# quickwit-oss/quickwit

Hardware: NVIDIA H100
Metric: docs_scored_per_sec (higher is better)
Workload: dtype f32+u32

## Files before the change

quickwit_b200/csrc/capi_engine.cpp:

```cpp
#include "engine.h"

#define QW_API_BEGIN try {
#define QW_API_END                                   \
  }                                                  \
  catch (const qw::Error& e) {                       \
    qw::set_last_error(e.what());                    \
    return e.code;                                   \
  }                                                  \
  catch (const std::exception& e) {                  \
    qw::set_last_error(e.what());                    \
    return QWGPU_EINTERNAL;                          \
  }

static qw::Engine& engine_of(qwgpu_ctx* ctx) {
  if (!ctx) qw::fail(QWGPU_EINVALID_ARG, "null context");
  if (!ctx->engine) qw::fail(QWGPU_ENODEVICE, "host-only context: no CUDA device bound (there is no CPU search path)");
  return *ctx->engine;
}

extern "C" {

int qwgpu_init(int device, qwgpu_ctx** out) {
  QW_API_BEGIN
  if (!out) qw::fail(QWGPU_EINVALID_ARG, "null out pointer");
// ... 56 lines not shown
int qwgpu_split_is_resident(qwgpu_ctx* ctx, const char* split_id) {
  if (!ctx || !ctx->engine || !split_id) return 0;
  std::lock_guard<std::mutex> g(ctx->engine->mu);
  return ctx->engine->splits.count(split_id) ? 1 : 0;
}

uint64_t qwgpu_resident_bytes(qwgpu_ctx* ctx) {
  if (!ctx || !ctx->engine) return 0;
  std::lock_guard<std::mutex> g(ctx->engine->mu);
  return ctx->engine->resident;
}

int qwgpu_split_search(qwgpu_ctx* ctx, uint32_t num_splits, const char* const* split_ids,
                       const uint8_t* const* plans, const size_t* plan_lens,
                       qwgpu_split_result* results, int* status) {
  QW_API_BEGIN
  qw::Engine& e = engine_of(ctx);
  std::vector<std::shared_ptr<qw::SplitDev>> sp(num_splits);
  std::vector<const uint8_t*> pl(plans, plans + num_splits);
  std::vector<size_t> ln(plan_lens, plan_lens + num_splits);
  for (uint32_t i = 0; i < num_splits; i++) sp[i] = e.find(split_ids[i]);
  std::vector<qw::SplitOutput> outs;
  qw::BatchStats st;
  e.search(sp, pl, ln, outs, st);
  std::string first_err;
  for (uint32_t i = 0; i < num_splits; i++) {
    qwgpu_split_result& r = results[i];
    memset(&r, 0, sizeof r);
    status[i] = outs[i].status;
    if (outs[i].status) { if (first_err.empty()) first_err = outs[i].error; continue; }
    r.num_hits = outs[i].num_hits;
    r.num_partial_hits = (uint32_t)outs[i].hits.size();
    r.num_agg_cells = (uint32_t)outs[i].cells.size();
    if (!outs[i].hits.empty()) {
      r.hits = (QwHit*)malloc(outs[i].hits.size() * sizeof(QwHit));
      memcpy(r.hits, outs[i].hits.data(), outs[i].hits.size() * sizeof(QwHit));
    }
    if (!outs[i].cells.empty()) {
      r.agg_cells = (QwAggCell*)malloc(outs[i].cells.size() * sizeof(QwAggCell));
      memcpy(r.agg_cells, outs[i].cells.data(), outs[i].cells.size() * sizeof(QwAggCell));
    }
    r.gpu_time_us = st.gpu_time_us;
    r.main_kernel_us = st.main_kernel_us;
    r.num_kernel_launches = st.launches;
    r.exact_fallbacks = st.exact_fallbacks;
    r.postings_scored = outs[i].postings_scored;
    r.algorithmic_bytes = outs[i].algorithmic_bytes;
    r.kernel_mask = st.kernel_mask;
    r.window_docs = st.window_docs;
    r.sample_stride = st.sample_stride;
    r.radix_passes = st.radix_passes;
    r.refined = st.refined;
  }
  if (!first_err.empty()) qw::set_last_error(first_err);
  return 0;
  QW_API_END
}

void qwgpu_split_result_free(qwgpu_split_result* r) {
  if (!r) return;
  free(r->hits);
  free(r->agg_cells);
  r->hits = nullptr;
  r->agg_cells = nullptr;
}

}
```

quickwit_b200/csrc/common.h:

```cpp
#pragma once
#include <cmath>
#include <cstdarg>
#include <cstdint>
#include <cstdio>
#include <cstdlib>
#include <cstring>
#include <stdexcept>
#include <string>
#include <vector>

#include "../../include/qwgpu.h"

namespace qw {

struct Error : std::runtime_error {
  int code;
  Error(int c, const std::string& m) : std::runtime_error(m), code(c) {}
};
[[noreturn]] inline void fail(int code, const char* fmt, ...) {
  char buf[1024];
  va_list ap;
  va_start(ap, fmt);
  vsnprintf(buf, sizeof buf, fmt, ap);
  va_end(ap);
  throw Error(code, buf);
}
void set_last_error(const std::string& msg);

inline uint64_t i64_to_u64(int64_t v) { return (uint64_t)v ^ (1ull << 63); }
inline int64_t u64_to_i64(uint64_t v) { return (int64_t)(v ^ (1ull << 63)); }
inline uint64_t f64_to_u64(double d) {
  uint64_t bits;
  memcpy(&bits, &d, 8);
  return (bits & (1ull << 63)) ? ~bits : (bits ^ (1ull << 63));
}
inline double u64_to_f64(uint64_t v) {
  uint64_t bits = (v & (1ull << 63)) ? (v ^ (1ull << 63)) : ~v;
  double d;
  memcpy(&d, &bits, 8);
  return d;
}

constexpr float BM25_K1 = 1.2f;
constexpr float BM25_B = 0.75f;
inline float bm25_idf(uint64_t doc_freq, uint64_t doc_count) {
  float x = ((float)(doc_count - doc_freq) + 0.5f) / ((float)doc_freq + 0.5f);
  return logf(1.0f + x);
}

struct ImageView {
  const uint8_t* base = nullptr;
  uint64_t len = 0;
  const QwImgHeader* hdr = nullptr;
  const QwImgField* fields = nullptr;
  const QwImgTerm* terms = nullptr;
  const QwImgColumn* columns = nullptr;
  const uint8_t* term_bytes = nullptr;
  const uint8_t* strings = nullptr;
  const uint8_t* data = nullptr;

  void open(const uint8_t* p, uint64_t n) {
    if (n < sizeof(QwImgHeader)) fail(QWGPU_EINVALID_ARG, "split image too small");
    const QwImgHeader* h = (const QwImgHeader*)p;
    if (h->magic != QW_IMG_MAGIC) fail(QWGPU_EINVALID_ARG, "bad split image magic");
    if (h->version != QW_IMG_VERSION) fail(QWGPU_EINVALID_ARG, "split image version %u (this library reads version %u)", h->version, QW_IMG_VERSION);
    if (h->total_len > n) fail(QWGPU_EINVALID_ARG, "split image truncated");
    const uint64_t tl = h->total_len;
    auto inside = [](uint64_t off, uint64_t count, uint64_t size, uint64_t limit) {
// ... 94 lines not shown
```

quickwit_b200/csrc/device_types.h:

```cpp
#pragma once
#include <stddef.h>
#include <stdint.h>

#include "../../include/qwgpu_format.h"

#ifndef QW_THREADS
#define QW_THREADS 512
#endif
#ifndef QW_MIN_BLOCKS_PER_SM
#define QW_MIN_BLOCKS_PER_SM 2
#endif
#define QW_WARPS (QW_THREADS / 32)
#define QW_MAX_INSTR 96
#define QW_MAX_DCOLS 16
#define QW_MAX_DAGGS 8
#define QW_MAX_LEVELS QW_MAX_PLAN_DEPTH
#define QW_MAX_TERMS 64
#define QW_BLK_TAB 160
#define QW_MAX_WBLK 512
#define QW_HIST_BINS 2048
#define QW_DIGIT_BITS 11
#define QW_KEY_BITS 192
#define QW_CAND_CAP 8192
#define QW_MAX_TOPK 4096
// ... 54 lines not shown

struct alignas(16) DKeySpec {
  uint32_t kind[2], order[2], col[2];
  uint32_t rbits[2];
  uint32_t hasbit[2];
  uint32_t doc_bits, total_bits;
  uint32_t top_mode;
  float score_scale;
  uint64_t raw_max[2];
  uint32_t narrow, sh_has[2], sh_r[2], sh_doc;
};
static_assert(sizeof(DKeySpec) % 16 == 0, "uint4-copied struct");
enum { QW_TOP_FULL = 0, QW_TOP_SCORE = 1, QW_TOP_COLUMN = 2, QW_TOP_DOC = 3 };

struct DThresh {
  uint64_t key[3];
  uint32_t prefix_bits;
  uint32_t above;
  uint32_t done;
  uint32_t matched;
};

struct DSplitPlan {
  uint64_t data_base;
  uint32_t num_docs, num_windows;
  uint32_t n_instr, instr_base;
  uint32_t n_cols, col_base;
  uint32_t n_aggs, agg_base;
  uint32_t n_terms, n_levels;
  uint32_t max_hits, scoring;
  uint32_t n_fn_slots, n_cells;
  uint32_t fused_score_root;
  uint32_t fast_aggs;
  uint32_t n_stat_cells, pad1;
  uint64_t fn_off[2];
  uint64_t bm25_tab[2];
  DKeySpec key;
  QwSearchAfter sa;
  uint64_t out_num_hits;
  uint64_t out_hist;
  uint64_t out_cand_count;
  uint64_t out_cands;
  uint64_t out_cells;
  uint64_t out_hits;
  uint64_t out_nhits;
};

static_assert(offsetof(DSplitPlan, key) % 16 == 0 && sizeof(DSplitPlan) % 16 == 0, "DKeySpec is read as uint4");

struct SmemLevel {
  uint32_t req, shd, nt, cnt, msum, ssum;
  uint32_t rsc, pad;
};
struct SmemLayout {
  uint32_t instr, cols, aggs, key, hitq;
  uint32_t rangeq;
  SmemLevel lvl[QW_MAX_LEVELS];
  uint32_t tmp, fn[2];
  uint32_t rng, blkrec, termblk, stage, hist, misc;
  uint32_t l0hist;
  uint32_t total;
};

struct KParams {
  const DSplitPlan* plans;
  const DInstr* instrs;
  const DCol* cols;
// ... 20 lines not shown
```

quickwit_b200/csrc/engine.cu:

```cuda
#include <algorithm>
#include <chrono>
#include <cmath>

#include "engine.h"
#include "kernels.cuh"
#include "union_kernel.cuh"
#include "phrase_kernel.cuh"
#include "driver_kernel.cuh"
#include "agg_kernel.cuh"

namespace qw {

#define CUDA_CHECK(expr)                                                                          \
  do {                                                                                            \
    cudaError_t _e = (expr);                                                                      \
    if (_e != cudaSuccess)                                                                        \
      fail((_e == cudaErrorNoDevice || _e == cudaErrorInsufficientDriver) ? QWGPU_ENODEVICE       \
                                                                           : QWGPU_EINTERNAL,     \
           "CUDA error %s at %s:%d: %s", cudaGetErrorName(_e), __FILE__, __LINE__,               \
           cudaGetErrorString(_e));                                                               \
  } while (0)

uint32_t id_to_fieldnorm(uint8_t id);

// ... 689 lines not shown
  if (rec_l0) L.l0hist = take(QW_HIST_BINS * 4);
  if (rangeq) L.rangeq = take(QW_WARPS * (32 + 32 * 4) * 2);
  L.total = off;
  return L;
}

static qwk::USmem make_union_layout(uint32_t W, bool hist, uint32_t budget) {
  qwk::USmem L;
  memset(&L, 0, sizeof L);
  uint32_t off = 0;
  auto take = [&](uint32_t bytes) { uint32_t o = off; off = (off + bytes + 15) & ~15u; return o; };
  L.score = take(W * 4);
  L.bars = take(8 * (2 * QU_SLOTS + QU_CHAIN));
  if (hist) L.hist = take(QW_HIST_BINS * 4);
  L.cands = take(QU_NCW * QU_CANDS * 8 + QU_NCW * 4);
  const uint32_t fixed = QU_MAXBLK * 16 + QU_MAX_TERMS * 16 + 32 + QU_PAD;
  uint32_t cap = budget > off + QU_SLOTS * (fixed + 2048) ? ((budget - off) / QU_SLOTS - fixed) & ~15u : 2048;
  if (const char* e = getenv("QWGPU_UCAP")) cap = (uint32_t)atoi(e) & ~15u;
  L.cap = cap;
  L.payload = 0;
  L.recs = cap + QU_PAD;
  L.ttab = L.recs + QU_MAXBLK * 16;
  L.hdr = L.ttab + QU_MAX_TERMS * 16;
  L.slot_stride = L.hdr + 48;
  L.slot0 = take(QU_SLOTS * L.slot_stride);
  L.total = off;
  return L;
}

void Engine::search(const std::vector<std::shared_ptr<SplitDev>>& sp, const std::vector<const uint8_t*>& plans,
                    const std::vector<size_t>& plan_lens, std::vector<SplitOutput>& outs, BatchStats& stats,
                    const MergeSpec* merge, std::vector<MergedHit>* merged, const GatherSpec* gather, std::vector<RankHeader>* rank_headers) {
  const uint32_t n_in = (uint32_t)sp.size();
  outs.assign(n_in, SplitOutput());
  static const bool trace = getenv("QWGPU_TRACE") != nullptr;
  using tclock = std::chrono::steady_clock;
  const auto t_begin = tclock::now();
  CUDA_CHECK(cudaSetDevice(device));
  std::vector<Lowered> low;
  std::vector<uint32_t> idx;
  low.reserve(n_in);
  for (uint32_t i = 0; i < n_in; i++) {
    try {
      if (!sp[i]) fail(QWGPU_ENOTFOUND, "split not registered");
      Lowered L;
      lower_plan(L, *sp[i], plans[i], plan_lens[i]);
      low.push_back(std::move(L));
      idx.push_back(i);
    } catch (const Error& e) {
      outs[i].status = e.code;
      outs[i].error = e.what();
    }
  }
  const uint32_t n = (uint32_t)low.size();
  if (n == 0) {
    if (merge && merged && gather && gather->allgather && gather->world > 1 && rank_headers && merge->k) {
      const size_t rec = 64 + (size_t)merge->k * sizeof(qwk::DMergedHit), W8 = (size_t)gather->world;
      uint8_t *d = nullptr;
      const size_t o_recv = 256 * ((rec + 255) / 256), o_fin = o_recv + 256 * ((W8 * rec + 255) / 256), o_cut = o_fin + 256 * ((16 + rec + 255) / 256), o_hd = o_cut + 1024, total = o_hd + W8 * 64;
      CUDA_CHECK(cudaMalloc(&d, total));
      cudaStream_t st0 = nullptr;
      CUDA_CHECK(cudaStreamCreateWithFlags(&st0, cudaStreamNonBlocking));
      CUDA_CHECK(cudaMemsetAsync(d, 0, total, st0));
      qwk::DRankHeader h;
      memset(&h, 0, sizeof h);
      h.attempted = gather->attempted; h.successful = gather->successful; h.n_failed = gather->n_failed;
      CUDA_CHECK(cudaMemcpyAsync(d, &h, sizeof h, cudaMemcpyHostToDevice, st0));
// ... 160 lines not shown
  fw_all[0] = fw_smp[0] = 0;
  for (uint32_t i = 0; i < n; i++) {
    uint32_t nw = low[i].P.num_windows, phase = stride > 1 ? i % stride : 0;
    fw_all[i + 1] = fw_all[i] + nw;
    if (use_union) nw = low[i].empty ? 0 : (low[i].P.num_docs + W_h - 1) / W_h;
    if (edge_sample) {
      uint32_t cnt = 0;
      for (uint32_t w = 0; w < nw; w++) {
        const bool edge = w == 0 || w + 1 == nw, strided = w % stride == phase;
        if (edge || strided) { sample_win.push_back(w | (edge ? 0x80000000u : 0u)); cnt++; }
      }
      fw_smp[i + 1] = fw_smp[i] + cnt;
    } else fw_smp[i + 1] = fw_smp[i] + (nw > phase ? (nw - phase + stride - 1) / stride : 0);
  }
  uint32_t n_phrases = 0, phrase_blocks = 0;
  for (auto& L : low)
    for (size_t k = 0; k < L.phrases.size(); k++) { n_phrases++; phrase_blocks += L.instrs[L.phrase_instr[k]].n; }
  auto al = [](size_t x) { return (x + 255) & ~(size_t)255; };
  size_t o_plans = 0, o_instr = al(o_plans + n * sizeof(DSplitPlan)), o_cols = al(o_instr + tot_instr * sizeof(DInstr)),
         o_aggs = al(o_cols + std::max(tot_cols, 1u) * sizeof(DCol)), o_fwa = al(o_aggs + std::max(tot_aggs, 1u) * sizeof(DAgg)),
         o_fws = al(o_fwa + (n + 1) * 4), o_bounds = al(o_fws + (n + 1) * 4), o_rank = al(o_bounds + (size_t)tot_bounds * 8),
         o_smp = al(o_rank + (size_t)n * 4), o_phr = al(o_smp + sample_win.size() * 4), o_fwd = al(o_phr + (size_t)n_phrases * sizeof(DPhrase)),
         o_fwds = al(o_fwd + (use_driver ? (size_t)(n + 1) * 4 : 0)), blob_bytes = al(o_fwds + (use_driver ? (size_t)(n + 1) * 4 : 0));
  const bool do_merge = merge && merged && merge->k > 0 && any_topk && merge->rank.size() == n_in;
  uint32_t kmax = 1;
  for (auto& L : low) kmax = std::max(kmax, L.P.max_hits);
  size_t s_thr = 0, s_hist = al(s_thr + n * sizeof(DThresh)), s_state = al(s_hist + (size_t)n * QW_HIST_BINS * 4),
         s_ctr = al(s_state + (size_t)n * 4), s_wmax = al(s_ctr + 64 * 4), s_cand = al(s_wmax + (rec_l0 ? (size_t)fw_all[n] * 2 : 0)),
         s_hits = al(s_cand + (any_topk ? (size_t)n * QW_CAND_CAP * 24 : 0)),
         s_cut = al(s_hits + (do_merge ? (size_t)n * kmax * sizeof(QwHit) : 0)),
         s_grecv = al(s_cut + (size_t)std::max<uint32_t>(n, 64) * 4 + 1024),
         s_vblk = al(s_grecv + (gather && gather->world > 1 && do_merge ? (size_t)gather->world * (64 + (size_t)merge->k * sizeof(qwk::DMergedHit)) : 0)),
         scratch_bytes = al(s_vblk + (size_t)phrase_blocks * sizeof(VBlk));
  std::vector<size_t> out_off(n + 1);
  out_off[0] = 0;
  for (uint32_t i = 0; i < n; i++)
    out_off[i + 1] = al(out_off[i] + 32 + (do_merge ? 0 : (size_t)low[i].P.max_hits * sizeof(QwHit)) + (size_t)low[i].P.n_cells * sizeof(QwAggCell));
  const size_t o_merged = out_off[n];
  const size_t rec_bytes = do_merge ? 64 + (size_t)merge->k * sizeof(qwk::DMergedHit) : 0;
  const bool do_gather = do_merge && gather && gather->allgather && gather->world > 1 && rank_headers;
  const size_t o_ghdr = al(o_merged + rec_bytes), o_final = al(o_ghdr + (do_gather ? (size_t)gather->world * 64 : 0));
  size_t out_bytes = do_merge ? (do_gather ? al(o_final + 16 + (size_t)merge->k * sizeof(qwk::DMergedHit)) : al(o_merged + rec_bytes)) : out_off[n];

  static const int max_in_flight = getenv("QWGPU_MAX_IN_FLIGHT") ? std::max(1, atoi(getenv("QWGPU_MAX_IN_FLIGHT"))) : 16;
  CallSlot* slot = nullptr;
  {
    std::unique_lock<std::mutex> g(mu);
    cv_admit.wait(g, [&] { return admitted < max_in_flight; });
    admitted++;
    if (!free_slots.empty()) { slot = free_slots.back(); free_slots.pop_back(); }
  }
  struct Admit {
    Engine* e;
    ~Admit() {
      { std::lock_guard<std::mutex> g(e->mu); e->admitted--; }
      e->cv_admit.notify_one();
    }
  } admit{this};
  if (!slot) {
    slot = new CallSlot();
    CUDA_CHECK(cudaStreamCreateWithFlags(&slot->stream, cudaStreamNonBlocking));
    CUDA_CHECK(cudaEventCreate(&slot->ev0));
    CUDA_CHECK(cudaEventCreate(&slot->ev1));
    CUDA_CHECK(cudaEventCreate(&slot->ev2));
    CUDA_CHECK(cudaEventCreate(&slot->ev3));
    CUDA_CHECK(cudaEventCreateWithFlags(&slot->ev_block, cudaEventBlockingSync | cudaEventDisableTiming));
  }
  struct Release {
    Engine* e; CallSlot* s;
    ~Release() {
      cudaStreamSynchronize(s->stream);
      e->in_flight.fetch_sub(1);
      std::lock_guard<std::mutex> g(e->mu);
      e->free_slots.push_back(s);
    }
  } rel{this, slot};
  in_flight.fetch_add(1);
  static const uint32_t spin_limit = getenv("QWGPU_SPIN_LIMIT") ? (uint32_t)atoi(getenv("QWGPU_SPIN_LIMIT")) : std::max(2u, std::thread::hardware_concurrency() / 4);
  auto wait_stream = [&]() {
    if (in_flight.load(std::memory_order_relaxed) > (int)spin_limit) {
      CUDA_CHECK(cudaEventRecord(slot->ev_block, slot->stream));
      CUDA_CHECK(cudaEventSynchronize(slot->ev_block));
    } else CUDA_CHECK(cudaStreamSynchronize(slot->stream));
  };
  size_t want_blob, want_scratch, want_out;
  {
    std::lock_guard<std::mutex> g(mu);
    hw_blob = std::max(hw_blob, blob_bytes); hw_scratch = std::max(hw_scratch, scratch_bytes); hw_out = std::max(hw_out, out_bytes);
    auto sized = [](size_t hw, size_t need) { return hw <= ((size_t)64 << 20) ? hw : need; };
    want_blob = sized(hw_blob, blob_bytes); want_scratch = sized(hw_scratch, scratch_bytes); want_out = sized(hw_out, out_bytes);
  }
  slot->ensure(want_blob, want_scratch, want_out);
  cudaStream_t st = slot->stream;

  uint32_t phr_done = 0, phr_blocks_done = 0;
  for (uint32_t i = 0; i < n; i++) {
    DSplitPlan& P = low[i].P;
    if (P.fast_aggs && (((size_t)P.n_cells * 4 + 7) & ~(size_t)7) + (size_t)P.n_stat_cells * 24 > stage_bytes_for(W)) P.fast_aggs = 0;
    uint8_t* ob = slot->d_out + out_off[i];
    P.out_num_hits = (uint64_t)ob;
    P.out_nhits = (uint64_t)(ob + 16);
    P.out_cand_count = (uint64_t)(ob + 20);
    P.out_hits = do_merge ? (uint64_t)(slot->d_scratch + s_hits + (size_t)i * kmax * sizeof(QwHit)) : (uint64_t)(ob + 32);
    P.out_cells = (uint64_t)(ob + 32 + (do_merge ? 0 : (size_t)P.max_hits * sizeof(QwHit)));
    P.out_hist = (uint64_t)(slot->d_scratch + s_hist + (size_t)i * QW_HIST_BINS * 4);
    P.out_cands = (uint64_t)(slot->d_scratch + s_cand + (size_t)i * QW_CAND_CAP * 24);
    for (size_t k = 0; k < low[i].phrases.size(); k++) {
      DPhrase& ph = low[i].phrases[k];
      DInstr& pin = low[i].instrs[low[i].phrase_instr[k]];
      ph.first_work = phr_blocks_done;
      ph.out = (uint64_t)(slot->d_scratch + s_vblk + (size_t)phr_blocks_done * sizeof(VBlk));
      pin.a = ph.out;
      phr_blocks_done += pin.n;
      memcpy(slot->h_blob + o_phr + (size_t)phr_done++ * sizeof(DPhrase), &ph, sizeof ph);
    }
    memcpy(slot->h_blob + o_plans + i * sizeof(DSplitPlan), &P, sizeof P);
    memcpy(slot->h_blob + o_instr + P.instr_base * sizeof(DInstr), low[i].instrs.data(), P.n_instr * sizeof(DInstr));
    if (P.n_cols) memcpy(slot->h_blob + o_cols + P.col_base * sizeof(DCol), low[i].cols.data(), P.n_cols * sizeof(DCol));
    if (P.fast_aggs)
      for (DAgg& d : low[i].aggs)
        if (d.kind == QW_AGG_HISTOGRAM) d.bounds = (uint64_t)(slot->d_blob + o_bounds) + (low[i].bounds_base + d.bounds) * 8;
    if (P.n_aggs) memcpy(slot->h_blob + o_aggs + P.agg_base * sizeof(DAgg), low[i].aggs.data(), P.n_aggs * sizeof(DAgg));
    if (!low[i].bounds.empty()) memcpy(slot->h_blob + o_bounds + (size_t)low[i].bounds_base * 8, low[i].bounds.data(), low[i].bounds.size() * 8);
  }
  if (do_merge) for (uint32_t i = 0; i < n; i++) ((uint32_t*)(slot->h_blob + o_rank))[i] = merge->rank[idx[i]];
  if (!sample_win.empty()) memcpy(slot->h_blob + o_smp, sample_win.data(), sample_win.size() * 4);
  if (use_driver) { memcpy(slot->h_blob + o_fwd, fw_drv.data(), (n + 1) * 4); memcpy(slot->h_blob + o_fwds, fw_dsm.data(), (n + 1) * 4); }
  memcpy(slot->h_blob + o_fwa, fw_all.data(), (n + 1) * 4);
  memcpy(slot->h_blob + o_fws, fw_smp.data(), (n + 1) * 4);
  CUDA_CHECK(cudaMemcpyAsync(slot->d_blob, slot->h_blob, blob_bytes, cudaMemcpyHostToDevice, st));
  stats.h2d_bytes += blob_bytes;

  KParams kp;
  memset(&kp, 0, sizeof kp);
  kp.plans = (const DSplitPlan*)(slot->d_blob + o_plans);
  kp.instrs = (const DInstr*)(slot->d_blob + o_instr);
  kp.cols = (const DCol*)(slot->d_blob + o_cols);
// ... 62 lines not shown
      if (dynamic_work && n_ctr < 64) u.work_ctr = (uint32_t*)(slot->d_scratch + s_ctr) + n_ctr++;
#ifdef QU_PROFILE
      static unsigned long long* d_prof = nullptr;
      if (!d_prof) CUDA_CHECK(cudaMalloc(&d_prof, 16 * 8));
      if (mode == qwk::MODE_COLLECT) { CUDA_CHECK(cudaMemsetAsync(d_prof, 0, 16 * 8, st)); u.prof = d_prof; }
#endif
      const uint32_t ugrid = std::min<uint32_t>(q.total_work, (uint32_t)(sm_count * QU_MINB) - (do_gather ? 4u : 0u));
      if (mode == qwk::MODE_HIST) qwk::k_union<qwk::MODE_HIST><<<ugrid, QU_THREADS, u.sm.total, st>>>(u);
      else qwk::k_union<qwk::MODE_COLLECT><<<ugrid, QU_THREADS, u.sm.total, st>>>(u);
#ifdef QU_PROFILE
      if (u.prof && getenv("QWGPU_UPROF")) {
        unsigned long long h[16];
        CUDA_CHECK(cudaMemcpyAsync(h, d_prof, sizeof h, cudaMemcpyDeviceToHost, st));
        wait_stream();
        const double np = (double)ugrid, nc = (double)h[15];
        fprintf(stderr, "[uprof] producer/CTA: total %.0f cyc, empty-wait %.0f, phaseA %.0f, window(A+B) %.0f, windows %.1f, slots %.1f | consumer/warp: total %.0f, full-wait %.0f, chain-wait %.0f (end-of-window %.0f), sweep %.0f, block-loop %.0f, blocks %.1f\n",
                h[0] / np, h[1] / np, h[2] / np, h[3] / np, h[4] / np, h[5] / np, h[8] / nc, h[9] / nc, h[10] / nc, h[11] / nc, h[12] / nc, h[13] / nc, h[14] / nc);
      }
#endif
      stats.launches++;
      stats.kernel_mask |= QWGPU_KERNEL_UNION;
      return;
    }
    uint32_t grid = std::min<uint32_t>(q.total_work, (uint32_t)(sm_count * occ));
    if (mode == qwk::MODE_HIST && all_union && old_union && level == 0 && !use_prefix) qwk::k_window<qwk::MODE_HIST, true><<<grid, QW_THREADS, lay.total, st>>>(q);
    else if (mode == qwk::MODE_HIST) qwk::k_window<qwk::MODE_HIST, false><<<grid, QW_THREADS, lay.total, st>>>(q);
    else if (all_union && old_union) qwk::k_window<qwk::MODE_COLLECT, true><<<grid, QW_THREADS, lay.total, st>>>(q);
    else qwk::k_window<qwk::MODE_COLLECT, false><<<grid, QW_THREADS, lay.total, st>>>(q);
    stats.launches++;
    stats.kernel_mask |= QWGPU_KERNEL_WINDOW;
  };
  const uint32_t sel_smem = 3 * 8 * QW_CAND_CAP;
  auto run_collect = [&](uint32_t flags) {
    if (!(flags & F_CANDS_ONLY)) CUDA_CHECK(cudaMemsetAsync(slot->d_out, 0, out_bytes, st));
    CUDA_CHECK(cudaEventRecord(slot->ev2, st));
    launch_window(qwk::MODE_COLLECT, false, 0, 0, flags);
    CUDA_CHECK(cudaEventRecord(slot->ev3, st));
    if (any_topk) { qwk::k_select<<<n, 1024, sel_smem, st>>>(kp.plans, kp.cols); stats.launches++; }
    if (do_merge) {
      uint32_t* d_cut = (uint32_t*)(slot->d_scratch + s_cut);
      const qwk::SrcSplits src{kp.plans, (const uint32_t*)(slot->d_blob + o_rank), do_gather ? 1u : 0u};
      qwk::k_merge_prep<qwk::SrcSplits><<<1, 1024, 0, st>>>(src, n, merge->k, merge->order1, merge->order2, d_cut);
      const uint64_t threads = (uint64_t)n * kmax * 32;
      qwk::k_merge<qwk::SrcSplits><<<(uint32_t)((threads + 255) / 256), 256, 0, st>>>(src, d_cut, n, kmax, merge->k, merge->order1, merge->order2,
                                                          (qwk::DMergedHit*)(slot->d_out + o_merged + 64), (uint32_t*)(slot->d_out + o_merged));
      stats.launches += 2;
    }
    const size_t back = do_gather ? o_ghdr : out_bytes;
    CUDA_CHECK(cudaMemcpyAsync(slot->h_out, slot->d_out, back, cudaMemcpyDeviceToHost, st));
    stats.d2h_bytes += back;
  };
  std::vector<uint32_t> state(n, 0);
  auto verify = [&]() -> bool {
    bool all = true;
    for (uint32_t i = 0; i < n; i++) {
      state[i] = 0;
      if (low[i].P.max_hits == 0) continue;
      const uint8_t* ob = slot->h_out + out_off[i];
      uint64_t eligible = ((const uint64_t*)ob)[1];
      uint32_t cand = *(const uint32_t*)(ob + 20);
      if (cand > QW_CAND_CAP || cand < std::min<uint64_t>(low[i].P.max_hits, eligible)) { state[i] = 1; all = false; }
    }
    return all;
  };

  const auto t_staged = tclock::now();
  CUDA_CHECK(cudaEventRecord(slot->ev0, st));
// ... 75 lines not shown
    qwk::k_rank_header<<<1, 32, 0, st>>>(kp.plans, n, (qwk::DRankHeader*)(slot->d_out + o_merged), gather->attempted, gather->successful, gather->n_failed);
    uint8_t* g_recv = slot->d_scratch + s_grecv;
    if (gather->allgather(gather->comm, slot->d_out + o_merged, g_recv, rec_bytes, (void*)st)) fail(QWGPU_EINTERNAL, "ncclAllGather failed");
    const qwk::SrcGathered gsrc{g_recv, (uint32_t)rec_bytes, 64u};
    uint32_t* g_cut = d_cut + std::max<uint32_t>(n, 64);
    qwk::k_merge_prep<qwk::SrcGathered><<<1, 1024, 0, st>>>(gsrc, (uint32_t)gather->world, merge->k, merge->order1, merge->order2, g_cut);
    const uint64_t gthreads = (uint64_t)gather->world * merge->k * 32;
    qwk::k_merge<qwk::SrcGathered><<<(uint32_t)((gthreads + 255) / 256), 256, 0, st>>>(gsrc, g_cut, (uint32_t)gather->world, merge->k, merge->k, merge->order1, merge->order2,
                                                                                    (qwk::DMergedHit*)(slot->d_out + o_final + 16), (uint32_t*)(slot->d_out + o_final));
    CUDA_CHECK(cudaMemcpy2DAsync(slot->d_out + o_ghdr, 64, g_recv, rec_bytes, 64, (size_t)gather->world, cudaMemcpyDeviceToDevice, st));
    CUDA_CHECK(cudaMemcpyAsync(slot->h_out + o_ghdr, slot->d_out + o_ghdr, out_bytes - o_ghdr, cudaMemcpyDeviceToHost, st));
    CUDA_CHECK(cudaEventRecord(slot->ev1, st));
    wait_stream();
    stats.launches += 4;
    stats.d2h_bytes += out_bytes - o_ghdr;
  }
  CUDA_CHECK(cudaGetLastError());
  {
    float ms = 0;
    cudaEventElapsedTime(&ms, slot->ev0, slot->ev1);
    stats.gpu_time_us += ms * 1000.f;
    add_main();
    stats.main_kernel_us = main_ms * 1000.f;
  }

  const auto t_searched = tclock::now();
  for (uint32_t i = 0; i < n; i++) {
    SplitOutput& o = outs[idx[i]];
    const DSplitPlan& P = low[i].P;
    const uint8_t* ob = slot->h_out + out_off[i];
    o.num_hits = ((const uint64_t*)ob)[0];
    uint32_t nh = *(const uint32_t*)(ob + 16);
    if (!do_merge) {
      o.hits.assign((const QwHit*)(ob + 32), (const QwHit*)(ob + 32) + nh);
      if (P.key.kind[0] == QW_SORT_DOCID) for (auto& h : o.hits) { h.flags &= ~1u; h.v1 = 0; }
    }
    const QwAggCell* c = (const QwAggCell*)(ob + 32 + (do_merge ? 0 : (size_t)P.max_hits * sizeof(QwHit)));
    o.cells.assign(c, c + P.n_cells);
    for (auto& cell : o.cells) cell.min_mapped = ~cell.min_mapped;
    o.postings_scored = low[i].postings;
    uint64_t bytes = low[i].alg_bytes;
    const SplitDev& s = *sp[idx[i]];
    auto col_bytes = [&](uint32_t c, uint64_t probes) {
      const QwImgColumn& ic = s.view.columns[c];
      uint64_t full = ((uint64_t)ic.num_vals * ic.bits + 7) / 8;
      return std::min<uint64_t>(probes * ((ic.bits + 7) / 8), full);
    };
    uint64_t driver = low[i].min_required_df == ~0ull ? P.num_docs : low[i].min_required_df;
    for (auto& rc : low[i].range_cols) bytes += col_bytes(rc.first, driver);
    const QwPlanHeader* ph = (const QwPlanHeader*)plans[idx[i]];
    for (int k = 0; k < 2; k++)
      if (ph->sort[k].kind == QW_SORT_COLUMN && ph->sort[k].column != 0xFFFFFFFFu && P.max_hits) bytes += col_bytes(ph->sort[k].column, o.num_hits);
    const QwAggNode* an = (const QwAggNode*)(plans[idx[i]] + sizeof(QwPlanHeader) + (size_t)ph->num_nodes * sizeof(QwPlanNode));
    for (uint32_t a = 0; a < ph->num_aggs; a++) if (an[a].column != 0xFFFFFFFFu) bytes += col_bytes(an[a].column, o.num_hits);
    o.algorithmic_bytes = bytes;
  }
  if (do_gather) {
    const uint32_t nm = *(const uint32_t*)(slot->h_out + o_final);
    const qwk::DMergedHit* mh = (const qwk::DMergedHit*)(slot->h_out + o_final + 16);
    merged->resize(nm);
    const bool by_doc = low[0].P.key.kind[0] == QW_SORT_DOCID;
    for (uint32_t j = 0; j < nm; j++) {
      MergedHit& m = (*merged)[j];
      m.hit = mh[j].hit; m.split = mh[j].split; m.pad = 0;
      if (by_doc) { m.hit.flags &= ~1u; m.hit.v1 = 0; }
    }
    rank_headers->resize(gather->world);
    memcpy(rank_headers->data(), slot->h_out + o_ghdr, (size_t)gather->world * 64);
  } else if (do_merge) {
    const uint32_t nm = *(const uint32_t*)(slot->h_out + o_merged);
// ... 19 lines not shown
```

quickwit_b200/csrc/engine.h:

```cpp
#pragma once
#include <condition_variable>
#include <atomic>
#include <map>
#include <memory>
#include <mutex>
#include <thread>
#include <string>
#include <vector>

#include "common.h"

namespace qw {

struct SplitDev {
  std::string id;
  std::vector<uint8_t> dir;
  ImageView view;
  uint8_t* d_data = nullptr;
  float* d_tabs = nullptr;
  uint64_t data_len = 0;
  uint64_t last_use = 0;
  int state = 1;
  std::string load_error;
  ~SplitDev();
};

struct CallSlot;

struct SplitOutput {
  uint64_t num_hits = 0;
  std::vector<QwHit> hits;
  std::vector<QwAggCell> cells;
  int status = 0;
  std::string error;
  uint64_t postings_scored = 0;
  uint64_t algorithmic_bytes = 0;
};
struct MergeSpec {
  uint32_t k = 0;
  uint32_t order1 = QW_ORDER_DESC, order2 = QW_ORDER_DESC;
  std::vector<uint32_t> rank;
};
struct MergedHit {
  QwHit hit;
  uint32_t split;
  uint32_t pad;
};
struct RankHeader {
  uint32_t n_hits, pad;
  uint64_t num_hits, attempted, successful, n_failed, reserved[3];
};
struct GatherSpec {
  int world = 1, rank = 0;
  int (*allgather)(void* comm, const void* send, void* recv, size_t bytes, void* stream) = nullptr;
  void* comm = nullptr;
  uint64_t attempted = 0, successful = 0, n_failed = 0;
};
struct BatchStats {
  float gpu_time_us = 0;
  float main_kernel_us = 0;
  uint32_t launches = 0;
  uint32_t exact_fallbacks = 0;
  uint64_t h2d_bytes = 0, d2h_bytes = 0;
  uint32_t kernel_mask = 0;
// ... 49 lines not shown
```

quickwit_b200/csrc/kernels.cuh:

```cuda
#pragma once
#include <cuda_runtime.h>

#include "device_types.h"

namespace qwk {

extern __shared__ __align__(16) uint8_t qw_smem[];

struct Key {
  uint64_t w0, w1, w2;
};

__device__ __forceinline__ bool key_ge(const Key& a, const Key& b) {
  if (a.w0 != b.w0) return a.w0 > b.w0;
  if (a.w1 != b.w1) return a.w1 > b.w1;
  return a.w2 >= b.w2;
}
__device__ __forceinline__ bool key_lt(const Key& a, const Key& b) { return !key_ge(a, b); }

__device__ __forceinline__ void key_put(Key& k, uint32_t pos, uint64_t v, uint32_t nbits) {
  if (nbits == 0) return;
  const uint32_t sh = 192u - pos - nbits, w = sh >> 6, s = sh & 63u;
  const uint64_t lo = v << s, hi = s ? v >> (64u - s) : 0ull;
  if (w == 0) { k.w2 |= lo; k.w1 |= hi; }
  else if (w == 1) { k.w1 |= lo; k.w0 |= hi; }
  else k.w0 |= lo;
}
__device__ __forceinline__ uint64_t key_get(const Key& k, uint32_t pos, uint32_t nbits) {
  if (nbits == 0) return 0;
  const uint32_t sh = 192u - pos - nbits, w = sh >> 6, s = sh & 63u;
  const uint64_t lo = w == 0 ? k.w2 : (w == 1 ? k.w1 : k.w0);
  const uint64_t hi = w == 0 ? k.w1 : (w == 1 ? k.w0 : 0ull);
  const uint64_t v = s ? ((lo >> s) | (hi << (64u - s))) : lo;
  return nbits >= 64 ? v : (v & ((1ull << nbits) - 1));
}
__device__ __forceinline__ uint32_t key_digit(const Key& k, uint32_t level) {
  uint32_t o = level * QW_DIGIT_BITS, word = o >> 6, sh = o & 63;
  uint64_t hi = word == 0 ? k.w0 : (word == 1 ? k.w1 : k.w2);
  uint64_t lo = word == 0 ? k.w1 : (word == 1 ? k.w2 : 0ull);
  uint64_t v = sh ? ((hi << sh) | (lo >> (64 - sh))) : hi;
  return (uint32_t)(v >> (64 - QW_DIGIT_BITS));
}
__device__ __forceinline__ bool key_prefix_eq(const Key& a, const uint64_t* t, uint32_t bits) {
  if (bits == 0) return true;
  uint64_t x0 = a.w0 ^ t[0], x1 = a.w1 ^ t[1], x2 = a.w2 ^ t[2];
  if (bits <= 64) return (x0 >> (64 - bits)) == 0;
  if (x0) return false;
  if (bits <= 128) return (x1 >> (128 - bits)) == 0;
  if (x1) return false;
  return (x2 >> (192 - bits)) == 0;
}

__device__ __forceinline__ uint32_t f32_ordered(float f) {
  uint32_t b = __float_as_uint(f);
  return (b & 0x80000000u) ? ~b : (b | 0x80000000u);
}
__device__ __forceinline__ uint64_t f64_to_u64_dev(double d) {
  uint64_t b = (uint64_t)__double_as_longlong(d);
  return (b & (1ull << 63)) ? ~b : (b ^ (1ull << 63));
}
__device__ __forceinline__ double mapped_to_f64(uint32_t type, uint64_t m) {
  switch (type) {
    case QW_COL_U64: case QW_COL_BOOL: case QW_COL_STR: return (double)m;
    case QW_COL_I64: case QW_COL_DATETIME: return (double)(long long)(m ^ (1ull << 63));
    default: {
      uint64_t bits = (m & (1ull << 63)) ? (m ^ (1ull << 63)) : ~m;
      return __longlong_as_double((long long)bits);
    }
  }
}

__device__ __forceinline__ uint64_t col_raw(const uint8_t* base, const DCol& c, uint64_t idx) {
  if (c.bits == 0) return 0;
  const uint64_t* w = (const uint64_t*)(base + c.values_off);
  uint64_t bitpos = idx * c.bits, wi = bitpos >> 6;
  uint32_t sh = (uint32_t)(bitpos & 63);
  uint64_t v = __ldg(w + wi) >> sh;
  if (sh + c.bits > 64) v |= __ldg(w + wi + 1) << (64 - sh);
  return c.bits == 64 ? v : (v & ((1ull << c.bits) - 1));
}
__device__ __forceinline__ void col_range(const uint8_t* base, const DCol& c, uint32_t d, uint64_t& a, uint64_t& b) {
  if (c.card == QW_CARD_FULL) { a = d; b = (uint64_t)d + 1; return; }
  const uint8_t* ix = base + c.index_off;
  if (c.card == QW_CARD_OPTIONAL) {
    const uint64_t* present = (const uint64_t*)ix;
    const uint32_t* rank = (const uint32_t*)(ix + 8ull * c.nwords64);
    uint64_t word = __ldg(present + (d >> 6));
    if (!((word >> (d & 63)) & 1)) { a = b = 0; return; }
    a = __ldg(rank + (d >> 6)) + __popcll(word & ((1ull << (d & 63)) - 1));
    b = a + 1;
    return;
  }
// ... 209 lines not shown
    const bool in = (uint32_t)j < nvalid && rel[j] < wlen;
    inmask |= (in ? 1u : 0u) << j;
    f[j] = (has_fn && in) ? fn[rel[j]] : 1u;
  }
#pragma unroll
  for (int j = 0; j < 4; j++) {
    const uint32_t t = tf[j];
    float tfn = 0.0f;
    if ((inmask >> j) & 1) {
      if (t < QW_TFF_ROWS) tfn = __ldg(tab + 256 + t * 256 + f[j]);
      else { float tff = (float)t; tfn = __fdiv_rn(tff, __fadd_rn(tff, __ldg(tab + f[j]))); }
    }
    contrib[j] = __fmul_rn(tg.weight, tfn);
  }
}

struct DocKey {
  Key key;
  bool eligible;
};
__device__ __forceinline__ uint32_t score_lin(const DKeySpec& ks, float score, bool desc) {
  const float x = __fmul_rn(score, ks.score_scale);
  const uint32_t l = x >= 1023.0f ? 1023u : (x > 0.0f ? (uint32_t)x : 0u);
  return desc ? l : 1023u - l;
}
__device__ __forceinline__ DocKey doc_key(const DSplitPlan& P, const DKeySpec& ks, const DCol* cols, const uint8_t* base, uint32_t doc, float score) {
  uint32_t has[2] = {0, 0};
  uint64_t v[2] = {0, 0}, r[2] = {0, 0};
#pragma unroll
  for (int i = 0; i < 2; i++) {
    const bool desc = ks.order[i] == QW_ORDER_DESC;
    if (ks.kind[i] == QW_SORT_SCORE) {
      has[i] = 1;
      v[i] = f64_to_u64_dev((double)score);
      const uint32_t o = f32_ordered(score);
      r[i] = desc ? o : ~o;
      if (i == 0) r[i] |= (uint64_t)score_lin(ks, score, desc) << 32;
    } else if (ks.kind[i] == QW_SORT_COLUMN && ks.col[i] != 0xFFFFFFFFu) {
      const DCol& c = cols[ks.col[i]];
      uint64_t a, b;
      col_range(base, c, doc, a, b);
      if (a != b) {
        has[i] = 1;
        const uint64_t raw = col_raw(base, c, a);
        v[i] = c.min_value + c.gcd * raw;
        r[i] = desc ? raw : ks.raw_max[i] - raw;
      }
    }
  }
  const bool desc1 = ks.order[0] == QW_ORDER_DESC;
  const uint32_t docmask = ks.doc_bits >= 32 ? 0xFFFFFFFFu : ((1u << ks.doc_bits) - 1);
  DocKey out;
  out.key = Key{0, 0, 0};
  const uint32_t docr = desc1 ? doc : docmask - doc;
  if (ks.narrow) {
    out.key.w0 = ((uint64_t)(has[0] & ks.hasbit[0]) << ks.sh_has[0]) | (r[0] << ks.sh_r[0]) |
                 ((uint64_t)(has[1] & ks.hasbit[1]) << ks.sh_has[1]) | (r[1] << ks.sh_r[1]) |
                 ((uint64_t)(ks.doc_bits ? docr : 0u) << ks.sh_doc);
  } else {
    uint32_t pos = 0;
#pragma unroll
    for (int i = 0; i < 2; i++) {
      if (ks.hasbit[i]) { key_put(out.key, pos, has[i], 1); pos++; }
      key_put(out.key, pos, r[i], ks.rbits[i]);
      pos += ks.rbits[i];
    }
    key_put(out.key, pos, docr, ks.doc_bits);
// ... 1175 lines not shown
          if (act) other = Key{b0[tid ^ stride], b1[tid ^ stride], b2[tid ^ stride]};
          pb ^= 1;
        } else if (act) {
          other.w0 = __shfl_xor_sync(0xFFFFFFFFu, mine.w0, stride);
          other.w1 = __shfl_xor_sync(0xFFFFFFFFu, mine.w1, stride);
          other.w2 = __shfl_xor_sync(0xFFFFFFFFu, mine.w2, stride);
        }
        const bool want_larger = ((tid & stride) == 0) == ((tid & size) == 0);
        if (act && want_larger == key_lt(mine, other)) mine = other;
      }
    }
    __syncthreads();
    if (act) { k0[tid] = mine.w0; k1[tid] = mine.w1; k2[tid] = mine.w2; }
    __syncthreads();
  } else
  for (uint32_t size = 2; size <= N; size <<= 1) {
    for (uint32_t stride = size >> 1; stride > 0; stride >>= 1) {
      for (uint32_t i = tid; i < (N >> 1); i += 1024) {
        uint32_t pos = 2 * i - (i & (stride - 1));
        uint32_t q = pos + stride;
        bool desc = (pos & size) == 0;
        Key a{k0[pos], k1[pos], k2[pos]}, b{k0[q], k1[q], k2[q]};
        bool a_lt_b = key_lt(a, b);
        bool b_lt_a = key_lt(b, a);
        if (desc ? a_lt_b : b_lt_a) {
          k0[pos] = b.w0; k1[pos] = b.w1; k2[pos] = b.w2;
          k0[q] = a.w0; k1[q] = a.w1; k2[q] = a.w2;
        }
      }
      __syncthreads();
    }
  }
  const uint32_t out_n = m < K ? m : K;
  QwHit* hits = (QwHit*)P.out_hits;
  const DKeySpec& ks = P.key;
  const DCol* cols = all_cols + P.col_base;
  const uint32_t docmask = ks.doc_bits >= 32 ? 0xFFFFFFFFu : ((1u << ks.doc_bits) - 1);
  for (uint32_t i = tid; i < out_n; i += 1024) {
    const Key k{k0[i], k1[i], k2[i]};
    uint32_t pos = 0, has[2];
    uint64_t r[2];
#pragma unroll
    for (int f = 0; f < 2; f++) {
      has[f] = ks.hasbit[f] ? (uint32_t)key_get(k, pos, 1) : 0u;
      pos += ks.hasbit[f];
      r[f] = key_get(k, pos, ks.rbits[f]);
      pos += ks.rbits[f];
    }
    const uint32_t docr = (uint32_t)key_get(k, pos, ks.doc_bits);
    QwHit hh;
    hh.doc_id = ks.order[0] == QW_ORDER_DESC ? docr : docmask - docr;
    hh.flags = has[0] | (has[1] << 1);
    hh.score = 0.0f;
    hh.reserved = 0;
    uint64_t v[2] = {0, 0};
#pragma unroll
    for (int f = 0; f < 2; f++) {
      if (!has[f]) continue;
      const bool desc = ks.order[f] == QW_ORDER_DESC;
      if (ks.kind[f] == QW_SORT_SCORE) {
        uint32_t o = (uint32_t)r[f];
        if (!desc) o = ~o;
        const uint32_t bits = (o & 0x80000000u) ? (o & 0x7FFFFFFFu) : ~o;
        hh.score = __uint_as_float(bits);
        v[f] = f64_to_u64_dev((double)hh.score);
      } else {
        const DCol& c = cols[ks.col[f]];
        v[f] = c.min_value + c.gcd * (desc ? r[f] : ks.raw_max[f] - r[f]);
      }
    }
    hh.v1 = v[0];
    hh.v2 = v[1];
    hits[i] = hh;
  }
  if (tid == 0) *(uint32_t*)P.out_nhits = out_n;
}


struct MKey {
  uint64_t v1, v2, tie;
  uint32_t has;
};
__device__ __forceinline__ MKey merge_key(const QwHit& h, uint32_t rank, uint32_t o1, uint32_t o2) {
  MKey k;
  const uint32_t has1 = h.flags & 1u, has2 = (h.flags >> 1) & 1u;
  k.has = has1 << 1 | has2;
  k.v1 = has1 ? (o1 == QW_ORDER_DESC ? h.v1 : ~h.v1) : 0ull;
  k.v2 = has2 ? (o2 == QW_ORDER_DESC ? h.v2 : ~h.v2) : 0ull;
  const uint64_t t = ((uint64_t)rank << 32) | h.doc_id;
  k.tie = o1 == QW_ORDER_DESC ? t : ~t;
  return k;
}
__device__ __forceinline__ bool mkey_gt(const MKey& a, const MKey& b) {
  const uint32_t a1 = a.has >> 1, b1 = b.has >> 1;
  if (a1 != b1) return a1 > b1;
  if (a.v1 != b.v1) return a.v1 > b.v1;
  const uint32_t a2 = a.has & 1u, b2 = b.has & 1u;
  if (a2 != b2) return a2 > b2;
  if (a.v2 != b.v2) return a.v2 > b.v2;
  return a.tie > b.tie;
}
struct DMergedHit {
  QwHit hit;
  uint32_t split, pad;
};
struct SrcSplits {
// ... 127 lines not shown
```

Before: 158.7 billion.

## Emit packed sort keys from GPU and decode hits on host into owned buffer

In the non-merge path the top-k kernel now writes compact packed sort-key words instead of full QwHit structs, and the host decodes them with a shared host/device decoder. This shrinks device-to-host output, and the memset now clears only the header and cell region. Hits go into a malloc-backed HitBuf that the C API hands to callers without a second copy. Decoding moves to the host CPU and adds per-hit work there, and hits_as_keys takes over the former padding field.

New measurement: 163.1 billion (median of 6 runs). +2.8%, better.

```diff
diff --git a/quickwit_b200/csrc/capi_engine.cpp b/quickwit_b200/csrc/capi_engine.cpp
--- a/quickwit_b200/csrc/capi_engine.cpp
+++ b/quickwit_b200/csrc/capi_engine.cpp
@@ -112,10 +112,7 @@
     r.num_hits = outs[i].num_hits;
     r.num_partial_hits = (uint32_t)outs[i].hits.size();
     r.num_agg_cells = (uint32_t)outs[i].cells.size();
-    if (!outs[i].hits.empty()) {
-      r.hits = (QwHit*)malloc(outs[i].hits.size() * sizeof(QwHit));
-      memcpy(r.hits, outs[i].hits.data(), outs[i].hits.size() * sizeof(QwHit));
-    }
+    r.hits = outs[i].hits.release();
     if (!outs[i].cells.empty()) {
       r.agg_cells = (QwAggCell*)malloc(outs[i].cells.size() * sizeof(QwAggCell));
       memcpy(r.agg_cells, outs[i].cells.data(), outs[i].cells.size() * sizeof(QwAggCell));
diff --git a/quickwit_b200/csrc/common.h b/quickwit_b200/csrc/common.h
--- a/quickwit_b200/csrc/common.h
+++ b/quickwit_b200/csrc/common.h
@@ -10,6 +10,7 @@
 #include <vector>
 
 #include "../../include/qwgpu.h"
+#include "hit_decode.h"
 
 namespace qw {
 
@@ -29,11 +30,6 @@
 
 inline uint64_t i64_to_u64(int64_t v) { return (uint64_t)v ^ (1ull << 63); }
 inline int64_t u64_to_i64(uint64_t v) { return (int64_t)(v ^ (1ull << 63)); }
-inline uint64_t f64_to_u64(double d) {
-  uint64_t bits;
-  memcpy(&bits, &d, 8);
-  return (bits & (1ull << 63)) ? ~bits : (bits ^ (1ull << 63));
-}
 inline double u64_to_f64(uint64_t v) {
   uint64_t bits = (v & (1ull << 63)) ? (v ^ (1ull << 63)) : ~v;
   double d;
diff --git a/quickwit_b200/csrc/device_types.h b/quickwit_b200/csrc/device_types.h
--- a/quickwit_b200/csrc/device_types.h
+++ b/quickwit_b200/csrc/device_types.h
@@ -110,7 +110,8 @@
   uint32_t n_fn_slots, n_cells;
   uint32_t fused_score_root;
   uint32_t fast_aggs;
-  uint32_t n_stat_cells, pad1;
+  uint32_t n_stat_cells;
+  uint32_t hits_as_keys;
   uint64_t fn_off[2];
   uint64_t bm25_tab[2];
   DKeySpec key;
diff --git a/quickwit_b200/csrc/engine.cu b/quickwit_b200/csrc/engine.cu
--- a/quickwit_b200/csrc/engine.cu
+++ b/quickwit_b200/csrc/engine.cu
@@ -745,7 +745,8 @@
                     const std::vector<size_t>& plan_lens, std::vector<SplitOutput>& outs, BatchStats& stats,
                     const MergeSpec* merge, std::vector<MergedHit>* merged, const GatherSpec* gather, std::vector<RankHeader>* rank_headers) {
   const uint32_t n_in = (uint32_t)sp.size();
-  outs.assign(n_in, SplitOutput());
+  outs.clear();
+  outs.resize(n_in);
   static const bool trace = getenv("QWGPU_TRACE") != nullptr;
   using tclock = std::chrono::steady_clock;
   const auto t_begin = tclock::now();
@@ -972,15 +973,18 @@
          s_grecv = al(s_cut + (size_t)std::max<uint32_t>(n, 64) * 4 + 1024),
          s_vblk = al(s_grecv + (gather && gather->world > 1 && do_merge ? (size_t)gather->world * (64 + (size_t)merge->k * sizeof(qwk::DMergedHit)) : 0)),
          scratch_bytes = al(s_vblk + (size_t)phrase_blocks * sizeof(VBlk));
-  std::vector<size_t> out_off(n + 1);
+  auto al16 = [](size_t x) { return (x + 15) & ~(size_t)15; };
+  std::vector<size_t> out_off(n + 1), key_off(n + 1);
   out_off[0] = 0;
+  for (uint32_t i = 0; i < n; i++) out_off[i + 1] = al(out_off[i] + 32 + (size_t)low[i].P.n_cells * sizeof(QwAggCell));
+  key_off[0] = out_off[n];
   for (uint32_t i = 0; i < n; i++)
-    out_off[i + 1] = al(out_off[i] + 32 + (do_merge ? 0 : (size_t)low[i].P.max_hits * sizeof(QwHit)) + (size_t)low[i].P.n_cells * sizeof(QwAggCell));
+    key_off[i + 1] = al16(key_off[i] + (do_merge ? 0 : (size_t)low[i].P.max_hits * 4 * qw::key_words32(low[i].P.key)));
   const size_t o_merged = out_off[n];
   const size_t rec_bytes = do_merge ? 64 + (size_t)merge->k * sizeof(qwk::DMergedHit) : 0;
   const bool do_gather = do_merge && gather && gather->allgather && gather->world > 1 && rank_headers;
   const size_t o_ghdr = al(o_merged + rec_bytes), o_final = al(o_ghdr + (do_gather ? (size_t)gather->world * 64 : 0));
-  size_t out_bytes = do_merge ? (do_gather ? al(o_final + 16 + (size_t)merge->k * sizeof(qwk::DMergedHit)) : al(o_merged + rec_bytes)) : out_off[n];
+  size_t out_bytes = do_merge ? (do_gather ? al(o_final + 16 + (size_t)merge->k * sizeof(qwk::DMergedHit)) : al(o_merged + rec_bytes)) : key_off[n];
 
   static const int max_in_flight = getenv("QWGPU_MAX_IN_FLIGHT") ? std::max(1, atoi(getenv("QWGPU_MAX_IN_FLIGHT"))) : 16;
   CallSlot* slot = nullptr;
@@ -1041,8 +1045,9 @@
     P.out_num_hits = (uint64_t)ob;
     P.out_nhits = (uint64_t)(ob + 16);
     P.out_cand_count = (uint64_t)(ob + 20);
-    P.out_hits = do_merge ? (uint64_t)(slot->d_scratch + s_hits + (size_t)i * kmax * sizeof(QwHit)) : (uint64_t)(ob + 32);
-    P.out_cells = (uint64_t)(ob + 32 + (do_merge ? 0 : (size_t)P.max_hits * sizeof(QwHit)));
+    P.out_hits = do_merge ? (uint64_t)(slot->d_scratch + s_hits + (size_t)i * kmax * sizeof(QwHit)) : (uint64_t)(slot->d_out + key_off[i]);
+    P.hits_as_keys = do_merge ? 0 : 1;
+    P.out_cells = (uint64_t)(ob + 32);
     P.out_hist = (uint64_t)(slot->d_scratch + s_hist + (size_t)i * QW_HIST_BINS * 4);
     P.out_cands = (uint64_t)(slot->d_scratch + s_cand + (size_t)i * QW_CAND_CAP * 24);
     for (size_t k = 0; k < low[i].phrases.size(); k++) {
@@ -1171,7 +1176,7 @@
   };
   const uint32_t sel_smem = 3 * 8 * QW_CAND_CAP;
   auto run_collect = [&](uint32_t flags) {
-    if (!(flags & F_CANDS_ONLY)) CUDA_CHECK(cudaMemsetAsync(slot->d_out, 0, out_bytes, st));
+    if (!(flags & F_CANDS_ONLY)) CUDA_CHECK(cudaMemsetAsync(slot->d_out, 0, do_merge ? out_bytes : out_off[n], st));
     CUDA_CHECK(cudaEventRecord(slot->ev2, st));
     launch_window(qwk::MODE_COLLECT, false, 0, 0, flags);
     CUDA_CHECK(cudaEventRecord(slot->ev3, st));
@@ -1313,10 +1318,11 @@
     o.num_hits = ((const uint64_t*)ob)[0];
     uint32_t nh = *(const uint32_t*)(ob + 16);
     if (!do_merge) {
-      o.hits.assign((const QwHit*)(ob + 32), (const QwHit*)(ob + 32) + nh);
+      qw::decode_hits(qw::make_hit_decoder(P.key, low[i].cols.data()), (const uint32_t*)(slot->h_out + key_off[i]),
+                      qw::key_words32(P.key), nh, o.hits.alloc(nh));
       if (P.key.kind[0] == QW_SORT_DOCID) for (auto& h : o.hits) { h.flags &= ~1u; h.v1 = 0; }
     }
-    const QwAggCell* c = (const QwAggCell*)(ob + 32 + (do_merge ? 0 : (size_t)P.max_hits * sizeof(QwHit)));
+    const QwAggCell* c = (const QwAggCell*)(ob + 32);
     o.cells.assign(c, c + P.n_cells);
     for (auto& cell : o.cells) cell.min_mapped = ~cell.min_mapped;
     o.postings_scored = low[i].postings;
diff --git a/quickwit_b200/csrc/engine.h b/quickwit_b200/csrc/engine.h
--- a/quickwit_b200/csrc/engine.h
+++ b/quickwit_b200/csrc/engine.h
@@ -4,6 +4,7 @@
 #include <map>
 #include <memory>
 #include <mutex>
+#include <new>
 #include <thread>
 #include <string>
 #include <vector>
@@ -27,9 +28,42 @@
 
 struct CallSlot;
 
+struct HitBuf {
+  HitBuf() = default;
+  HitBuf(const HitBuf&) = delete;
+  HitBuf& operator=(const HitBuf&) = delete;
+  HitBuf(HitBuf&& o) noexcept : p(o.p), n(o.n) { o.p = nullptr; o.n = 0; }
+  HitBuf& operator=(HitBuf&& o) noexcept { if (this != &o) { free(p); p = o.p; n = o.n; o.p = nullptr; o.n = 0; } return *this; }
+  ~HitBuf() { free(p); }
+  QwHit* alloc(size_t k) {
+    free(p);
+    p = nullptr;
+    n = 0;
+    if (k) {
+      p = (QwHit*)malloc(k * sizeof(QwHit));
+      if (!p) throw std::bad_alloc();
+      n = k;
+    }
+    return p;
+  }
+  QwHit* release() { QwHit* r = p; p = nullptr; n = 0; return r; }
+  size_t size() const { return n; }
+  bool empty() const { return n == 0; }
+  QwHit* data() { return p; }
+  const QwHit* data() const { return p; }
+  QwHit& operator[](size_t i) { return p[i]; }
+  const QwHit& operator[](size_t i) const { return p[i]; }
+  QwHit* begin() { return p; }
+  QwHit* end() { return p + n; }
+
+ private:
+  QwHit* p = nullptr;
+  size_t n = 0;
+};
+
 struct SplitOutput {
   uint64_t num_hits = 0;
-  std::vector<QwHit> hits;
+  HitBuf hits;
   std::vector<QwAggCell> cells;
   int status = 0;
   std::string error;
diff --git a/quickwit_b200/csrc/hit_decode.h b/quickwit_b200/csrc/hit_decode.h
--- /dev/null
+++ b/quickwit_b200/csrc/hit_decode.h
@@ -0,0 +1,128 @@
+#pragma once
+#include <stdint.h>
+#include <string.h>
+
+#include "device_types.h"
+
+#ifdef __CUDACC__
+#define QW_HD __host__ __device__ __forceinline__
+#else
+#define QW_HD inline
+#endif
+
+namespace qw {
+
+QW_HD uint64_t f64_to_u64(double d) {
+#ifdef __CUDA_ARCH__
+  const uint64_t bits = (uint64_t)__double_as_longlong(d);
+#else
+  uint64_t bits;
+  memcpy(&bits, &d, 8);
+#endif
+  return (bits & (1ull << 63)) ? ~bits : (bits ^ (1ull << 63));
+}
+
+QW_HD float f32_from_bits(uint32_t b) {
+#ifdef __CUDA_ARCH__
+  return __uint_as_float(b);
+#else
+  float f;
+  memcpy(&f, &b, 4);
+  return f;
+#endif
+}
+
+QW_HD uint32_t key_words32(const DKeySpec& ks) { return (ks.total_bits + 31u) / 32u; }
+
+struct KeyField {
+  uint64_t mask;
+  uint32_t w, s;
+};
+QW_HD KeyField key_field_at(uint32_t pos, uint32_t nbits) {
+  KeyField f;
+  const uint32_t sh = nbits ? 192u - pos - nbits : 0u;
+  f.w = sh >> 6;
+  f.s = sh & 63u;
+  f.mask = nbits == 0 ? 0ull : (nbits >= 64 ? ~0ull : ((1ull << nbits) - 1));
+  return f;
+}
+QW_HD uint64_t key_get(const KeyField& f, uint64_t w0, uint64_t w1, uint64_t w2) {
+  const uint64_t lo = f.w == 0 ? w2 : (f.w == 1 ? w1 : w0);
+  const uint64_t hi = f.w == 0 ? w1 : (f.w == 1 ? w0 : 0ull);
+  return ((lo >> f.s) | ((hi << 1) << (63u - f.s))) & f.mask;
+}
+
+struct HitDecoder {
+  KeyField has[2], r[2], doc;
+  uint32_t kind[2];
+  uint32_t desc[2];
+  uint32_t doc_desc, docmask;
+  uint64_t raw_max[2], min_value[2], gcd[2];
+};
+QW_HD HitDecoder make_hit_decoder(const DKeySpec& ks, const DCol* cols) {
+  HitDecoder d;
+  uint32_t pos = 0;
+  for (int f = 0; f < 2; f++) {
+    d.has[f] = key_field_at(pos, ks.hasbit[f]);
+    pos += ks.hasbit[f];
+    d.r[f] = key_field_at(pos, ks.rbits[f]);
+    pos += ks.rbits[f];
+    d.kind[f] = !ks.hasbit[f] ? (uint32_t)QW_SORT_NONE : (ks.kind[f] == QW_SORT_SCORE ? (uint32_t)QW_SORT_SCORE : (uint32_t)QW_SORT_COLUMN);
+    d.desc[f] = ks.order[f] == QW_ORDER_DESC ? 1u : 0u;
+    d.raw_max[f] = ks.raw_max[f];
+    d.min_value[f] = d.kind[f] == QW_SORT_COLUMN ? cols[ks.col[f]].min_value : 0;
+    d.gcd[f] = d.kind[f] == QW_SORT_COLUMN ? cols[ks.col[f]].gcd : 0;
+  }
+  d.doc = key_field_at(pos, ks.doc_bits);
+  d.doc_desc = ks.order[0] == QW_ORDER_DESC ? 1u : 0u;
+  d.docmask = ks.doc_bits >= 32 ? 0xFFFFFFFFu : ((1u << ks.doc_bits) - 1);
+  return d;
+}
+
+QW_HD QwHit decode_hit(const HitDecoder& d, uint64_t w0, uint64_t w1, uint64_t w2) {
+  QwHit hh;
+  const uint32_t docr = (uint32_t)key_get(d.doc, w0, w1, w2);
+  hh.doc_id = d.doc_desc ? docr : d.docmask - docr;
+  hh.flags = 0;
+  hh.score = 0.0f;
+  hh.reserved = 0;
+  uint64_t v[2] = {0, 0};
+  for (int f = 0; f < 2; f++) {
+    if (d.kind[f] == QW_SORT_NONE) continue;
+    const uint32_t has = (uint32_t)key_get(d.has[f], w0, w1, w2);
+    hh.flags |= has << f;
+    if (!has) continue;
+    const uint64_t r = key_get(d.r[f], w0, w1, w2);
+    if (d.kind[f] == QW_SORT_SCORE) {
+      uint32_t o = (uint32_t)r;
+      if (!d.desc[f]) o = ~o;
+      const uint32_t bits = (o & 0x80000000u) ? (o & 0x7FFFFFFFu) : ~o;
+      hh.score = f32_from_bits(bits);
+      v[f] = f64_to_u64((double)hh.score);
+    } else {
+      v[f] = d.min_value[f] + d.gcd[f] * (d.desc[f] ? r : d.raw_max[f] - r);
+    }
+  }
+  hh.v1 = v[0];
+  hh.v2 = v[1];
+  return hh;
+}
+
+inline void decode_hits(const HitDecoder& dec, const uint32_t* kw, uint32_t nw, uint32_t n, QwHit* out) {
+  const HitDecoder d = dec;
+  for (uint32_t j = 0; j < n; j++, kw += nw) {
+    uint64_t w0 = 0, w1 = 0, w2 = 0;
+    switch (nw) {
+      case 6: w2 |= kw[5];
+      case 5: w2 |= (uint64_t)kw[4] << 32;
+      case 4: w1 |= kw[3];
+      case 3: w1 |= (uint64_t)kw[2] << 32;
+      case 2: w0 |= kw[1];
+      case 1: w0 |= (uint64_t)kw[0] << 32;
+      default: break;
+    }
+    out[j] = decode_hit(d, w0, w1, w2);
+  }
+}
+
+}
diff --git a/quickwit_b200/csrc/kernels.cuh b/quickwit_b200/csrc/kernels.cuh
--- a/quickwit_b200/csrc/kernels.cuh
+++ b/quickwit_b200/csrc/kernels.cuh
@@ -2,6 +2,7 @@
 #include <cuda_runtime.h>
 
 #include "device_types.h"
+#include "hit_decode.h"
 
 namespace qwk {
 
@@ -25,14 +26,6 @@
   if (w == 0) { k.w2 |= lo; k.w1 |= hi; }
   else if (w == 1) { k.w1 |= lo; k.w0 |= hi; }
   else k.w0 |= lo;
-}
-__device__ __forceinline__ uint64_t key_get(const Key& k, uint32_t pos, uint32_t nbits) {
-  if (nbits == 0) return 0;
-  const uint32_t sh = 192u - pos - nbits, w = sh >> 6, s = sh & 63u;
-  const uint64_t lo = w == 0 ? k.w2 : (w == 1 ? k.w1 : k.w0);
-  const uint64_t hi = w == 0 ? k.w1 : (w == 1 ? k.w0 : 0ull);
-  const uint64_t v = s ? ((lo >> s) | (hi << (64u - s))) : lo;
-  return nbits >= 64 ? v : (v & ((1ull << nbits) - 1));
 }
 __device__ __forceinline__ uint32_t key_digit(const Key& k, uint32_t level) {
   uint32_t o = level * QW_DIGIT_BITS, word = o >> 6, sh = o & 63;
@@ -54,10 +47,6 @@
 __device__ __forceinline__ uint32_t f32_ordered(float f) {
   uint32_t b = __float_as_uint(f);
   return (b & 0x80000000u) ? ~b : (b | 0x80000000u);
-}
-__device__ __forceinline__ uint64_t f64_to_u64_dev(double d) {
-  uint64_t b = (uint64_t)__double_as_longlong(d);
-  return (b & (1ull << 63)) ? ~b : (b ^ (1ull << 63));
 }
 __device__ __forceinline__ double mapped_to_f64(uint32_t type, uint64_t m) {
   switch (type) {
@@ -333,7 +322,7 @@
     const bool desc = ks.order[i] == QW_ORDER_DESC;
     if (ks.kind[i] == QW_SORT_SCORE) {
       has[i] = 1;
-      v[i] = f64_to_u64_dev((double)score);
+      v[i] = qw::f64_to_u64((double)score);
       const uint32_t o = f32_ordered(score);
       r[i] = desc ? o : ~o;
       if (i == 0) r[i] |= (uint64_t)score_lin(ks, score, desc) << 32;
@@ -1575,46 +1564,21 @@
     }
   }
   const uint32_t out_n = m < K ? m : K;
-  QwHit* hits = (QwHit*)P.out_hits;
-  const DKeySpec& ks = P.key;
-  const DCol* cols = all_cols + P.col_base;
-  const uint32_t docmask = ks.doc_bits >= 32 ? 0xFFFFFFFFu : ((1u << ks.doc_bits) - 1);
-  for (uint32_t i = tid; i < out_n; i += 1024) {
-    const Key k{k0[i], k1[i], k2[i]};
-    uint32_t pos = 0, has[2];
-    uint64_t r[2];
-#pragma unroll
-    for (int f = 0; f < 2; f++) {
-      has[f] = ks.hasbit[f] ? (uint32_t)key_get(k, pos, 1) : 0u;
-      pos += ks.hasbit[f];
-      r[f] = key_get(k, pos, ks.rbits[f]);
-      pos += ks.rbits[f];
-    }
-    const uint32_t docr = (uint32_t)key_get(k, pos, ks.doc_bits);
-    QwHit hh;
-    hh.doc_id = ks.order[0] == QW_ORDER_DESC ? docr : docmask - docr;
-    hh.flags = has[0] | (has[1] << 1);
-    hh.score = 0.0f;
-    hh.reserved = 0;
-    uint64_t v[2] = {0, 0};
-#pragma unroll
-    for (int f = 0; f < 2; f++) {
-      if (!has[f]) continue;
-      const bool desc = ks.order[f] == QW_ORDER_DESC;
-      if (ks.kind[f] == QW_SORT_SCORE) {
-        uint32_t o = (uint32_t)r[f];
-        if (!desc) o = ~o;
-        const uint32_t bits = (o & 0x80000000u) ? (o & 0x7FFFFFFFu) : ~o;
-        hh.score = __uint_as_float(bits);
-        v[f] = f64_to_u64_dev((double)hh.score);
-      } else {
-        const DCol& c = cols[ks.col[f]];
-        v[f] = c.min_value + c.gcd * (desc ? r[f] : ks.raw_max[f] - r[f]);
-      }
-    }
-    hh.v1 = v[0];
-    hh.v2 = v[1];
-    hits[i] = hh;
+  if (P.hits_as_keys) {
+    const uint32_t nw = qw::key_words32(P.key);
+    uint32_t* out = (uint32_t*)P.out_hits;
+    for (uint32_t i = tid; i < out_n; i += 1024) {
+      const uint64_t w0 = k0[i], w1 = k1[i], w2 = k2[i];
+      for (uint32_t j = 0; j < nw; j++) {
+        const uint64_t w = j < 2 ? w0 : (j < 4 ? w1 : w2);
+        out[(size_t)i * nw + j] = (uint32_t)(w >> ((j & 1) ? 0 : 32));
+      }
+    }
+  } else {
+    QwHit* hits = (QwHit*)P.out_hits;
+    const DCol* cols = all_cols + P.col_base;
+    const qw::HitDecoder dec = qw::make_hit_decoder(P.key, cols);
+    for (uint32_t i = tid; i < out_n; i += 1024) hits[i] = qw::decode_hit(dec, k0[i], k1[i], k2[i]);
   }
   if (tid == 0) *(uint32_t*)P.out_nhits = out_n;
 }
```
